# juhotuho10/rust_GPU_raytracing

Hardware: AMD Instinct MI355X
Metric: Mray/s (primary+bounce) at 1920x1080, 8 bounces; 1/2/4/8-GPU scaling (higher is better)
Workload: dtype f32

## Files before the change

include/rt_abi.h:

```cpp
#ifndef RT_ABI_H
#define RT_ABI_H

#include <stddef.h>
#include <stdint.h>

#ifdef __cplusplus
extern "C" {
#endif

#if defined(__GNUC__)
#define RT_API __attribute__((visibility("default")))
#else
#define RT_API
#endif

#define RT_ABI_VERSION 12

#define RT_OK 0
#define RT_E_INVALID -1
#define RT_E_HIP -2
#define RT_E_NOMEM -3
#define RT_E_CAPACITY -4
#define RT_E_NODEVICE -5

// ... 334 lines not shown
RT_API int rt_pack_owned_output(rt_ctx* ctx, void* dst_device);
RT_API int rt_unpack_output(rt_ctx* ctx, const void* src_device, uint32_t src_rank, uint32_t world_size);
RT_API int rt_unpack_accumulation_ranks(rt_ctx* ctx, const void* src_device, uint64_t stride_px,
                                        uint32_t world_size, uint32_t skip_rank, uint32_t divisor);
RT_API int rt_unpack_output_ranks(rt_ctx* ctx, const void* src_device, uint64_t stride_px, uint32_t world_size,
                                  uint32_t skip_rank);

RT_API int rt_launch_config(rt_ctx* ctx, uint32_t* threads, uint32_t* blocks, uint32_t* lds_bytes,
                            uint32_t* scene_in_lds);

#define RT_PASS_PATH 1u
#define RT_PASS_PRIMARY 2u
#define RT_PASS_RESOLVE 4u
#define RT_PASS_BRUTE 8u
#define RT_PASS_BRUTE_STREAM 16u
RT_API int rt_last_launch_passes(rt_ctx* ctx, uint32_t* passes);

RT_API int rt_debug_counters(rt_ctx* ctx, uint64_t* out, uint32_t n);

RT_API int rt_debug_check_leaf_certificates(rt_ctx* ctx, uint32_t* mismatches, uint32_t* valid, uint32_t* total);

RT_API int rt_math_selftest(uint32_t which, uint64_t* mismatches, uint32_t* first_bad);

RT_API void* rt_stream(rt_ctx* ctx);

RT_API int rt_srgb_table(float out[256]);

typedef struct rt_group rt_group;

RT_API int rt_create_multi(const rt_create_info* info, const int32_t* devices, uint32_t n_devices, rt_group** out);
// ... 72 lines not shown
```

rust_gpu_raytracing_amd/_native.py:

```python
from __future__ import annotations

import ctypes
import os
from pathlib import Path

import numpy as np

from . import buffers as B

LIB_NAME = "librt_pathtrace.so"
LIB_PATH = Path(__file__).resolve().parent / LIB_NAME

RT_OK = 0
RT_E_INVALID = -1
RT_E_HIP = -2
RT_E_NOMEM = -3
RT_E_CAPACITY = -4
RT_E_NODEVICE = -5

_ERR_NAMES = {
    RT_E_INVALID: "RT_E_INVALID",
    RT_E_HIP: "RT_E_HIP",
    RT_E_NOMEM: "RT_E_NOMEM",
    RT_E_CAPACITY: "RT_E_CAPACITY",
# ... 218 lines not shown
    "rt_group_update_triangles": (ctypes.c_int, [_P, _P, _U32]),
    "rt_group_update_object_info": (ctypes.c_int, [_P, _P, _U32]),
    "rt_group_update_sub_object_info": (ctypes.c_int, [_P, _P, _U32]),
    "rt_group_update_materials": (ctypes.c_int, [_P, _P, _U32]),
    "rt_group_upload_textures": (ctypes.c_int, [_P, _P, _U32, _U32, _U32]),
    "rt_group_upload_env_map": (ctypes.c_int, [_P, _P, _U32, _U32]),
    "rt_group_ray_count": (ctypes.c_int, [_P, ctypes.POINTER(ctypes.c_uint64)]),
    "rt_group_reset_ray_count": (ctypes.c_int, [_P]),
    "rt_gather_frame": (ctypes.c_int, [_P, _U32, _U32]),
    "rt_group_read_output": (ctypes.c_int, [_P, _U32, _P]),
    "rt_group_read_accumulation": (ctypes.c_int, [_P, _U32, _P]),
}

RT_DEFAULT_FRAME_BATCH = 16
RT_PASS_PATH, RT_PASS_PRIMARY, RT_PASS_RESOLVE, RT_PASS_BRUTE, RT_PASS_BRUTE_STREAM = 1, 2, 4, 8, 16
RT_GROUP_COPY_TRANSPORT = 1
RT_GATHER_IMAGE = 0
RT_GATHER_ACCUMULATION = 1
RT_DISPLAY_ACCUMULATION, RT_DISPLAY_DENOISED, RT_DISPLAY_PLANE = 0, 1, 2
RT_TONE_LINEAR, RT_TONE_REINHARD, RT_TONE_ACES = 0, 1, 2
RT_ENCODE_NONE, RT_ENCODE_SRGB = 0, 1

_lib = None


def load_library(path: os.PathLike | str | None = None) -> ctypes.CDLL:
    global _lib
    if path is None:
        if _lib is not None:
            return _lib
# ... 51 lines not shown
```

rust_gpu_raytracing_amd/csrc/pathtrace.hip:

```cpp
#include <hip/hip_runtime.h>
#include <stdint.h>

#include <algorithm>

#include "rt_path_common.h"
#include "rt_sphere_walk.h"
#include "rt_walk.h"

#ifdef RT_ISA_MARKS
#define RT_ISA_MARK(name) asm volatile("; RT_MARK " name)
#else
#define RT_ISA_MARK(name)
#endif

#pragma clang fp contract(off)

using namespace rtk;

constexpr uint32_t kPrimaryThreads = 1024;

constexpr uint32_t kQueueStride = 64;

__device__ __forceinline__ uint32_t* sched_orders(const KernelArgs& ka) { return ka.sched + 2u * ka.owned_tiles; }
__device__ __forceinline__ uint32_t* sched_flags(const KernelArgs& ka) { return ka.sched + 4u * ka.owned_tiles; }

__device__ __forceinline__ uint32_t xcc_id() {
    return __builtin_amdgcn_s_getreg((3 << 11) | (0 << 6) | 20);
}

struct TileQueue {
    uint32_t stripe;
    uint32_t empty;
// ... 16 lines not shown
            open = (uint64_t)v * n_str + st < ka.queue_units;
        }
        const uint64_t m = __ballot(open);
        if (m == 0) {
            q.empty = 1u;
            return 0xffffffffu;
        }
        uint32_t st = q.stripe + 1u + (uint32_t)__builtin_ctzll(m);
        q.stripe = st >= n_str ? st - n_str : st;
        if (lane == 0) old = atomicAdd(ka.queue + q.stripe * kQueueStride, 1u);
        pos = (uint64_t)__builtin_amdgcn_readlane(old, 0) * n_str + q.stripe;
        if (pos < ka.queue_units) return (uint32_t)pos;
    }
}

__device__ __forceinline__ uint32_t unit_tile(const KernelArgs& ka, uint32_t pos, uint32_t& frame) {
    if (pos == 0xffffffffu) return pos;
    uint32_t q;
    if (!ka.frame_light) {
        frame = 0u;
        q = pos;
    } else if (ka.unit_tile_major) {
        q = pos / ka.frames;
        frame = pos - q * ka.frames;
    } else {
        frame = pos / ka.owned_tiles;
        q = pos - frame * ka.owned_tiles;
    }
    return ka.tile_order ? ka.tile_order[q] : q;
}

__device__ __forceinline__ void record_tile_cost(uint32_t* cost, bool fin, uint32_t tile, uint32_t n) {
    uint64_t m = __ballot(fin);
    while (m) {
// ... 102 lines not shown
    unsigned long long* diag;
    __device__ __forceinline__ void operator()(bool walk, bool at_leaf, uint32_t) const {
        const uint64_t act = __ballot(walk), lf = __ballot(at_leaf);
        if (act && (threadIdx.x & 63u) == (uint32_t)__builtin_ctzll(__ballot(true))) {
            atomicAdd(diag + 22, 1ull);
            atomicAdd(diag + 23, (unsigned long long)__popcll(act));
            if (lf) {
                atomicAdd(diag + 24, 1ull);
                atomicAdd(diag + 25, (unsigned long long)__popcll(lf));
            }
        }
    }
};
#endif

template <int kMode, uint32_t kThreads, bool kTris>
__global__ void __launch_bounds__(kThreads, 1) rt_pathtrace_kernel(KernelArgs ka) {
    extern __shared__ __attribute__((aligned(16))) unsigned char lds[];
    __shared__ uint32_t block_rays;

    const uint32_t tid = threadIdx.x;
    if (ka.launch_clock && tid == 0) atomicMax(ka.launch_clock, ~(unsigned long long)wall_clock64());
    float* l_srgb = reinterpret_cast<float*>(lds + ka.lds_srgb_offset);
    SceneView sv{ka.sphere_slots, ka.sphere_orig, ka.sphere_material, ka.sphere_bvh, ka.materials, nullptr,
                 ka.objects,      l_srgb,         ka.tri_bvh,     ka.tri_prims, kTris ? *ka.tri_extent : 0.0f,
                 ka.sub_objects};
    if constexpr (kTris && kMode <= 1) {
        if (ka.tri_qnodes) {
            const float4 g0 = ka.tri_qgrid[0], g1 = ka.tri_qgrid[1];
            if (g0.w != 0.0f) {
                sv.tri_q = ka.tri_qnodes;
                sv.qox = g0.x;
                sv.qoy = g0.y;
                sv.qoz = g0.z;
                sv.qsx = g1.x;
                sv.qsy = g1.y;
// ... 48 lines not shown
        if (ka.lds_sub_offset) {
            RtSubObject* l_sub = reinterpret_cast<RtSubObject*>(lds + ka.lds_sub_offset);
            for (uint32_t i = tid; i < ka.sub_object_count; i += kThreads) l_sub[i] = ka.sub_objects[i];
            sv.sub = l_sub;
        }
    }
    for (uint32_t i = tid; i < 256u; i += kThreads) l_srgb[i] = ka.srgb[i];
    float* l_cam = l_srgb + 256;
    if (tid < 16u) {
        l_cam[tid] = ka.inv_proj[tid];
        l_cam[16u + tid] = ka.inv_view[tid];
    }
    if (tid == 0) l_cam[32] = ka.aspect;
    __syncthreads();

    const bool accumulate = ka.accumulate == 1u;
    const uint32_t samples = accumulate ? ka.compute_per_frame : 1u;

    constexpr uint32_t kIdle = 0, kSetup = 1, kTrav = 2, kDone = 3, kPrimary = 4;
    uint32_t rays = 0;
    uint32_t lane_tile = 0;
    uint32_t lane_slot = 0;
    const bool frame_par = ka.frame_light != nullptr;
    uint32_t mode = kIdle;
    uint32_t index = 0, sample = 0, frame = 0;
    float4 pix = make_float4(0.f, 0.f, 0.f, 0.f);
    Path p;
    p.o = p.d = mk(0.f, 0.f, 0.f);
    p.light = p.contrib = f4{0.f, 0.f, 0.f, 0.f};
    p.seed = p.bounce = 0;
    TraceState ts;
    ts.inv = mk(0.f, 0.f, 0.f);
    ts.a4 = ts.a2 = 0.f;
    ts.node = 0;
    ts.phase = 2;
    ts.nan_hit = false;
    ts.sph = SphereHit{kF32Max, 0u, 0u};
    ts.tri = TriHit{kF32Max, 0u, 0u, 0u, false};
// ... 8 lines not shown
        if (accumulate) {
            const float div = (float)((ka.accumulation_index + frame) * ka.compute_per_frame);
            r = clamp01(pix.x / div);
            g = clamp01(pix.y / div);
            b = clamp01(pix.z / div);
            a = clamp01(pix.w / div);
        } else {
            r = clamp01(p.light.x);
            g = clamp01(p.light.y);
            b = clamp01(p.light.z);
            a = clamp01(p.light.w);
        }
        if (accumulate) ka.accum[index] = pix;
        ka.output[index] = pack_rgba8(r, g, b, a);
    };
    auto finish_sample = [&]() {
        if (frame_par) {
            const size_t slot = (size_t)(frame * samples + sample) * ((size_t)ka.owned_tiles * 64u) +
                                (size_t)lane_tile * 64u + lane_slot;
            ka.frame_light[slot] = make_float4(p.light.x, p.light.y, p.light.z, p.light.w);
            sample += 1;
            if (sample < samples) {
                start_sample(ka, index, random_index(), pixel_ray(ka, l_cam, index, index % ka.width, index / ka.width),
                             p);
                mode = primary_start();
            } else {
                mode = kIdle;
            }
            return;
        }
        sample += 1;
        if (accumulate) {
            pix.x = pix.x + p.light.x;
            pix.y = pix.y + p.light.y;
            pix.z = pix.z + p.light.z;
            pix.w = pix.w + p.light.w;
        }
        if (sample == samples && frame + 1u < ka.frames) {
            store_frame();
            frame += 1;
            sample = 0;
        }
        if (sample < samples) {
            start_sample(ka, index, random_index(), pixel_ray(ka, l_cam, index, index % ka.width, index / ka.width), p);
            mode = primary_start();
        } else {
            store_frame();
            mode = kIdle;
        }
    };

#ifdef RT_DIAG_TAIL
    const unsigned long long wave_t0 = realtime();
    unsigned long long wave_dry = 0;
#endif
    if (blockIdx.x == 0 && threadIdx.x < ka.queue_stripes) ka.queue_next[threadIdx.x * kQueueStride] = 0u;
    TileQueue queue{(xcc_id() + 8u * (blockIdx.x >> 3)) % ka.queue_stripes, 0u};
    uint32_t tile_frame = 0;
    uint32_t tile = unit_tile(ka, claim_tile(ka, queue), tile_frame);
    uint32_t next = 0;
#ifdef RT_DIAG
    unsigned long long iters = 0, trav_cyc = 0, steps = 0, step_lanes = 0, shade_cyc = 0, refill_cyc = 0,
                       setup_cyc = 0, leaf_cyc = 0, leaf_steps = 0;
    unsigned long long shade_passes = 0, shade_lanes = 0, miss_lanes = 0, glass_lanes = 0, spec_lanes = 0,
                       setup_passes = 0, setup_lanes = 0;
    const unsigned long long t_start = stamp();
#endif
    while (true) {
#ifdef RT_DIAG
        ++iters;
        const unsigned long long ts0 = stamp();
#endif
        bool fin = false;
        uint32_t fin_rays = 0;
// ... 13 lines not shown
        }
#endif
        if (mode == kDone) {
            const Hit h = trace_end<kTris>(sv, ka, p.o, p.d, ts);
#ifdef RT_DIAG
            {
                const bool miss = h.t == kF32Max;
                const RtMaterial dmat = sv.mat[min(h.material_index, ka.material_count - 1u)];
                miss_lanes += (unsigned long long)__popcll(__ballot(miss));
                glass_lanes += (unsigned long long)__popcll(__ballot(!miss && dmat.glass > 0.0f));
                spec_lanes += (unsigned long long)__popcll(__ballot(!miss && !(dmat.glass > 0.0f) && dmat.specular > 0.0f));
            }
#endif
            ++rays;
            RT_ISA_MARK("shade");
            if (shade<(kMode >= 1)>(sv, ka, p, h)) {
                fin = true;
                fin_rays = p.bounce + (p.bounce < ka.bounces ? 1u : 0u);
                finish_sample();
            } else {
                mode = kSetup;
            }
        }
        if (ka.tile_cost) record_tile_cost(ka.tile_cost, fin, lane_tile, fin_rays);
#ifdef RT_DIAG
        const unsigned long long ts1 = stamp();
        shade_cyc += ts1 - ts0;
#endif
        RT_ISA_MARK("refill");
        while (true) {
            const uint64_t need = __ballot(mode == kIdle);
            if (need == 0 || tile >= ka.owned_tiles) break;
            const uint32_t avail = 64u - next;
            if (mode == kIdle) {
                const uint32_t rank =
                    __builtin_amdgcn_mbcnt_hi((uint32_t)(need >> 32), __builtin_amdgcn_mbcnt_lo((uint32_t)need, 0u));
                if (rank < avail) {
                    const uint32_t slot = next + rank;
                    const uint32_t gt = tile * ka.world_size + ka.rank;
                    const uint32_t x = (gt % ka.tiles_x) * 8u + (slot & 7u);
                    const uint32_t y = (gt / ka.tiles_x) * 8u + (slot >> 3);
                    if (x < ka.width && y < ka.height) {
                        index = y * ka.width + x;
                        lane_tile = tile;
                        lane_slot = slot;
                        sample = 0;
                        frame = tile_frame;
                        mode = kSetup;
                        if (accumulate && !frame_par) pix = ka.accum[index];
                        start_sample(ka, index, random_index(), pixel_ray(ka, l_cam, index, x, y), p);
                        mode = primary_start();
                    }
                }
            }
            next += min((uint32_t)__popcll(need), avail);
            if (next == 64u) {
                tile = unit_tile(ka, claim_tile(ka, queue), tile_frame);
                next = 0;
            #ifdef RT_DIAG_TAIL
                if (tile >= ka.owned_tiles && wave_dry == 0) wave_dry = realtime();
#endif
            }
        }
#ifdef RT_DIAG
        const unsigned long long ts2 = stamp();
        refill_cyc += ts2 - ts1;
#endif
#ifdef RT_DIAG
        {
            const uint64_t sm = __ballot(mode == kSetup);
            if (sm) {
                ++setup_passes;
                setup_lanes += (unsigned long long)__popcll(sm);
            }
        }
#endif
        RT_ISA_MARK("setup");
        if (mode == kSetup) {
            while (mode == kSetup && p.bounce >= ka.bounces) finish_sample();
            if (mode == kSetup) {
                trace_begin<kTris>(sv, ka, p.o, p.d, ts);
                mode = ts.phase == 2 ? kDone : kTrav;
            }
        }
#ifdef RT_DIAG
        setup_cyc += stamp() - ts2;
#endif
        if (__ballot(mode != kIdle) == 0 && tile >= ka.owned_tiles) break;
        const bool draining = tile >= ka.owned_tiles;
        uint32_t thresh = draining ? 0u : ka.trav_threshold;
        uint32_t n_active = 64u, min_steps = 0u;
        if constexpr (kDrainDecouple<kMode, kTris>) {
            if (draining) {
                thresh = ka.drain_threshold;
                n_active = (uint32_t)__popcll(__ballot(mode == kTrav || mode == kDone));
// ... 178 lines not shown
        if (tid == 0) {
            sorter = atomicAdd(sched_flags(ka) + par, 1u);
            if (blockIdx.x == 0) sched_flags(ka)[par ^ 1u] = 0u;
        }
        __syncthreads();
        if (sorter == 0)
            sort_tiles_by_cost<kThreads>(ka.sched + (par ^ 1u) * n, sched_orders(ka) + (par ^ 1u) * n, n,
                                         reinterpret_cast<uint32_t*>(lds + ka.lds_srgb_offset));
    }
    if (ka.launch_clock) {
        __syncthreads();
        if (tid == 0) atomicMax(ka.launch_clock + 1, (unsigned long long)wall_clock64());
    }
}

#define RT_FOR_EACH_CONFIG(X)                                                                                   \
    X(0, 256, true) X(0, 512, true) X(0, 1024, true) X(1, 256, true) X(1, 512, true) X(1, 1024, true)          \
    X(2, 256, true) X(2, 512, true) X(2, 1024, true) X(0, 256, false) X(0, 512, false) X(0, 1024, false)       \
    X(1, 256, false) X(1, 512, false) X(1, 1024, false)

constexpr uint32_t kBruteThreads = 256;

__device__ __forceinline__ void brute_sub_triangles(const KernelArgs& ka, f3 o, f3 d, uint32_t first_tri,
                                                    uint32_t count, uint32_t oi, float& closest, TriHit& best) {
    for (uint32_t j = 0; j < count; ++j) {
        const uint32_t ti = min(first_tri + j, ka.triangle_count - 1u);
        const TriGeom g = load_tri(ka.triangles, ti);
        const float det = -dot(d, g.cn);
        const float inv_det = 1.0f / det;
        const f3 ao = o - g.a;
        const float dist = dot(ao, g.cn) * inv_det;
        if (dist < 0.0f || dist >= closest) continue;
        const f3 dao = cross(ao, d);
        const float v = -dot(g.ab, dao) * inv_det;
// ... 510 lines not shown
            }();
    }
}

namespace {
hipError_t allow_big_lds(const void* fn) {
    int dev = 0, max_optin = 0;
    hipError_t e = hipGetDevice(&dev);
    if (e != hipSuccess) return e;
    e = hipDeviceGetAttribute(&max_optin, hipDeviceAttributeSharedMemPerBlockOptin, dev);
    if (e != hipSuccess || max_optin <= 0) return hipSuccess;
    return hipFuncSetAttribute(fn, hipFuncAttributeMaxDynamicSharedMemorySize, max_optin - 256);
}
}

hipError_t rt_launch_pathtrace(const KernelArgs& ka, int mode, bool tris, uint32_t threads, size_t lds_bytes,
                               uint32_t blocks, hipStream_t stream) {
#define RT_LAUNCH(M, T, TR)                                                                                    \
    if (mode == M && threads == T && tris == TR) {                                                            \
        hipLaunchKernelGGL((rt_pathtrace_kernel<M, T, TR>), dim3(blocks), dim3(T), lds_bytes, stream, ka);    \
        return hipGetLastError();                                                                             \
    }
    RT_FOR_EACH_CONFIG(RT_LAUNCH)
#undef RT_LAUNCH
    return hipErrorInvalidValue;
}

size_t rt_brute_wf_tile_bytes(bool stream) {
    if (stream) return (size_t)kBruteThreads * kBruteHits * 4u;
    return 2u * (size_t)kBruteWfTileSubs * sizeof(RtSubObject) + (size_t)kBruteThreads * kBruteRays * kBruteHits * 2u;
}

uint32_t rt_brute_wf_chunk() { return kBruteChunk; }

hipError_t rt_launch_brute_wf(const KernelArgs& ka, bool tris, bool scalar_stream, size_t lds_bytes, uint32_t blocks,
// ... 26 lines not shown
        if (lds_bytes > 64u * 1024u) {                                                                         \
            hipError_t e = allow_big_lds(reinterpret_cast<const void*>(&rt_primary_kernel<M, TR, T, W>));     \
            if (e != hipSuccess) return e;                                                                     \
        }                                                                                                      \
        hipLaunchKernelGGL((rt_primary_kernel<M, TR, T, W>), dim3(blocks), dim3(T), lds_bytes, stream, ka);   \
        return hipGetLastError();                                                                              \
    }
    RT_PRIMARY(1, true, 64, 0) RT_PRIMARY(1, true, 128, 0) RT_PRIMARY(1, true, 256, 0) RT_PRIMARY(1, true, 256, 8)
    RT_PRIMARY(1, true, 512, 0) RT_PRIMARY(1, true, 1024, 0) RT_PRIMARY(2, true, 1024, 0)
#undef RT_PRIMARY
    return hipErrorInvalidValue;
}

constexpr int kDefaultWavesPerCu = 16;

hipError_t rt_pathtrace_pick_config(int mode, bool tris, size_t lds_bytes, size_t lds_bytes_per_thread,
                                    uint32_t force_threads, uint32_t waves_cap, uint32_t* threads,
                                    int* blocks_per_cu) {
    const int kTargetWavesPerCu = waves_cap ? (int)waves_cap : kDefaultWavesPerCu;
    int best_waves = -1;
#define RT_OCC(M, T, TR)                                                                                  \
    if (mode == M && tris == TR) {                                                                        \
        int n = 0;                                                                                        \
        hipError_t e = allow_big_lds(reinterpret_cast<const void*>(&rt_pathtrace_kernel<M, T, TR>));     \
        if (e != hipSuccess) return e;                                                                    \
        e = hipOccupancyMaxActiveBlocksPerMultiprocessor(&n, rt_pathtrace_kernel<M, T, TR>, T,           \
                                                         lds_bytes + (size_t)T * lds_bytes_per_thread);  \
        if (e != hipSuccess) return e;                                                                    \
        const int waves = std::min(n * (int)(T / 64), kTargetWavesPerCu);                                 \
        if (n > 0 && (force_threads ? force_threads == T : waves > best_waves)) {                         \
            best_waves = waves;                                                                           \
            *threads = T;                                                                                 \
            *blocks_per_cu = force_threads ? n : std::max(1, std::min(n, kTargetWavesPerCu / (int)(T / 64))); \
        }                                                                                                 \
    }
    RT_FOR_EACH_CONFIG(RT_OCC)
#undef RT_OCC
    if (best_waves <= 0) return hipErrorInvalidConfiguration;
    return hipSuccess;
}

// ... 227 lines not shown
```

rust_gpu_raytracing_amd/csrc/rt_abi.cpp:

```cpp
#include <hip/hip_runtime.h>

#include <algorithm>
#include <cmath>
#include <cstddef>
#include <cstdio>
#include <cstdlib>
#include <cstring>
#include <initializer_list>
#include <new>
#include <string>
#include <vector>

#include "rt_abi.h"
#include "rt_kernel_args.h"
#include "rt_query_schedule.h"
#include "rt_scene_math.h"
#include "sphere_bvh.h"
#include "tri_cone.h"
#include "tri_qnode.h"

hipError_t rt_launch_math_selftest(uint32_t which, unsigned long long* mismatches, uint32_t* first_bad,
                                   hipStream_t stream);
hipError_t rt_launch_pathtrace(const KernelArgs& ka, int mode, bool tris, uint32_t threads, size_t lds_bytes,
                               uint32_t blocks, hipStream_t stream);
hipError_t rt_pathtrace_pick_config(int mode, bool tris, size_t lds_bytes, size_t lds_bytes_per_thread,
                                    uint32_t force_threads, uint32_t waves_cap, uint32_t* threads,
                                    int* blocks_per_cu);
hipError_t rt_launch_edit(const float* model, const uint32_t* tri_object, const uint32_t* sub_object,
                          const uint2* object_tris, const rt_scene::Placement* place, uint32_t object_count,
                          uint32_t n_tri, uint32_t n_sub, RtTriangleHot* tris, float4* bounds, RtSubObject* subs,
                          RtObject* objects, hipStream_t stream);
hipError_t rt_launch_quantize_tri_nodes(const SphereBvhNode* nodes, uint32_t n, const uint32_t* src,
                                        const uint32_t* skip, uint32_t n_out, SphereBvhNode* out32, uint4* q,
                                        float4* grid, hipStream_t stream);
hipError_t rt_launch_refit(SphereBvhNode* nodes, const SubObjectPrim* prims, const RtSubObject* subs,
                           const uint32_t* order, const uint32_t* level_offsets, uint32_t n_levels, float* extent_out,
                           hipStream_t stream);
hipError_t rt_launch_tri_leafcert(const SubObjectPrim* prims, uint32_t n_prims, const RtSubObject* subs,
                                  const RtTriangleHot* tris, uint32_t n_tri, TriLeafCert* out, hipStream_t stream);
hipError_t rt_launch_tri_leaftris(const SubObjectPrim* prims, uint32_t n_prims, const RtTriangleHot* tris,
                                  uint32_t n_tri, uint4* out, hipStream_t stream);
hipError_t rt_launch_primary(const KernelArgs& ka, int mode, bool tris, size_t lds_bytes, uint32_t threads,
// ... 144 lines not shown
    hipEvent_t ev_aux_done = nullptr;
    hipEvent_t ev_primary = nullptr;
    bool aux_outstanding = false;
    bool primary_dirty = true;
    uint64_t batches = 0;
    bool batch_overlap = true;
    bool stage_subs = true;
    size_t batch_budget = 0;
    bool use_qnodes = true;
    bool qnodes_dirty = true;
    bool derived_octants = false, derived_qnodes = false;
    uint4* d_tri_qnodes = nullptr;
    float4* d_tri_qgrid = nullptr;
    size_t qnodes_cap = 0;
    bool batch_schedule = false;
    bool unit_tile_major = true;

    uint32_t cap_mat = 0, cap_sph = 0, cap_tri = 0, cap_obj = 0, cap_sub = 0;
    uint32_t n_mat_dev = 1, n_tri_dev = 1, n_sub_dev = 1;

    float4* d_rays = nullptr;
    float4* d_accum = nullptr;
    uint32_t* d_out = nullptr;
    unsigned long long* d_counter = nullptr;
    uint32_t* d_queue = nullptr;
    uint32_t queue_parity[2] = {0, 0};
    uint32_t queue_stripes = kQueueStripes;
    int n_cu = 0;
    bool force_global_scene = false;
    size_t occ_lds_bytes = 0;
    int occ_mode = -1;
    bool occ_tris = false;
    size_t occ_stack_pt = 0;
    int max_lds_mode = 2;
    int occ_blocks_per_cu = 0;
    uint32_t occ_threads = 0;
    uint32_t force_threads = 0;
    uint32_t waves_cap = 0;
    uint32_t trav_threshold = 0;
    uint32_t drain_threshold = kDefaultDrainThreshold;
    uint32_t drain_min_steps = kDefaultDrainMinSteps;
    uint32_t leaf_batch = 0;
    uint32_t tile_schedule = kDefaultTileSchedule;
    uint32_t* d_tile_sched[2] = {};
    uint64_t sched_launches[2] = {};
    uint32_t last_blocks = 0, last_lds = 0;
    uint32_t last_passes = 0;
// ... 1053 lines not shown
        ka.tri_leaftris = ctx->d_tri_ltris;
    }
    if (sl.mode == 2) {
        ka.lds_srgb_offset = (uint32_t)(sl.mode2_bytes - kLdsTailBytes);
        sl.lds_bytes = sl.mode2_bytes;
    } else if (sl.mode == 1) {
        ka.lds_srgb_offset = (uint32_t)(sl.mode1_bytes - kLdsTailBytes);
        sl.lds_bytes = sl.mode1_bytes;
    } else {
        ka.lds_srgb_offset = 0;
        sl.lds_bytes = kLdsTailBytes;
    }
    return RT_OK;
}

static int dispatch_batch(rt_ctx* ctx, uint32_t bounces, uint32_t frames) {
    const rt_params& p = ctx->params;
    {
        int rc = refresh_sphere_slots(ctx, p.sphere_count, p.object_count == 0);
        if (rc) return rc;
        rc = refresh_tri_accel(ctx, p.object_count);
        if (rc) return rc;
    }
    KernelArgs ka{};
    ka.camera_rays = ctx->d_rays;
    ka.accum = ctx->d_accum;
    ka.output = ctx->d_out;
    ka.ray_counter = ctx->d_counter;
    ka.diag = ctx->d_counter + 1;
    ka.queue_stripes = ctx->queue_stripes;
// ... 22 lines not shown
            RT_HIP(ctx, join_aux(ctx));
            RT_HIP(ctx, hipStreamSynchronize(ctx->stream));
            for (float4*& b : ctx->d_frame_light) {
                if (b) RT_HIP(ctx, hipFree(b));
                b = nullptr;
            }
            ctx->frame_light_cap = 0;
            for (float4*& b : ctx->d_frame_light) {
                const hipError_t ea = hipMalloc(reinterpret_cast<void**>(&b), want * sizeof(float4));
                if (ea != hipSuccess) return fail(ctx, RT_E_NOMEM, std::string("frame lights: ") + hipGetErrorString(ea));
            }
            ctx->frame_light_cap = want;
        }
        ka.queue_units = ctx->owned_tiles * frames;
        ka.unit_tile_major = ctx->unit_tile_major ? 1u : 0u;
    }

    SceneLaunch sl;
    scene_carve(ctx, ka, ctx->force_global_scene ? 0 : ctx->max_lds_mode, sl);
    const bool tris = sl.tris;
    const int mode = sl.mode;
    if (ctx->brute) {
        scene_carve_layouts(ctx, ka, 1, kLdsSceneBudget, ctx->force_global_scene ? 0 : ctx->max_lds_mode, sl);
        ka.lds_srgb_offset = (uint32_t)(sl.mode1_bytes - kLdsTailBytes);
        ka.lds_stack_offset = (uint32_t)al16(sl.mode1_bytes);
        const uint32_t samples = ka.accumulate == 1u ? ka.compute_per_frame : 1u;
        const uint64_t passes = (uint64_t)frames * samples;
        const bool scalar_stream = tris && ctx->brute == 2;
        const size_t lds = ka.lds_stack_offset + rt_brute_wf_tile_bytes(scalar_stream);
        int dev = 0, max_optin = 0;
        RT_HIP(ctx, hipGetDevice(&dev));
// ... 47 lines not shown
        ctx->last_blocks = blocks;
        ctx->last_passes = RT_PASS_BRUTE | (scalar_stream ? RT_PASS_BRUTE_STREAM : 0u);
        ctx->last_lds = (uint32_t)lds;
        ctx->occ_threads = 256;
        ctx->primary_dirty = true;
        return RT_OK;
    }
    {
        const int rc = scene_accel_args(ctx, ka, sl);
        if (rc) return rc;
    }
    const bool coop = sl.coop;
    const size_t mode1_bytes = sl.mode1_bytes, mode2_bytes = sl.mode2_bytes;
    size_t lds_bytes = sl.lds_bytes;
    const size_t lane_pt = coop ? (size_t)kLeafBatchWaveBytes / 64u : 0u;
    if (ctx->occ_blocks_per_cu == 0 || ctx->occ_lds_bytes != lds_bytes || ctx->occ_mode != mode ||
        ctx->occ_tris != tris || ctx->occ_stack_pt != lane_pt) {
        int per_cu = 0;
        uint32_t threads = 0;
        hipError_t oe = rt_pathtrace_pick_config(mode, tris, lds_bytes, lane_pt, ctx->force_threads, ctx->waves_cap,
                                                 &threads, &per_cu);
        if (oe != hipSuccess) return hip_fail(ctx, "rt_pathtrace_pick_config (occupancy query)", oe);
        ctx->occ_blocks_per_cu = per_cu;
        ctx->occ_threads = threads;
        ctx->occ_lds_bytes = lds_bytes;
        ctx->occ_mode = mode;
        ctx->occ_tris = tris;
        ctx->occ_stack_pt = lane_pt;
    }
    ka.lds_leafbatch_offset = (uint32_t)al16(lds_bytes);
    if (coop) lds_bytes = ka.lds_leafbatch_offset + (size_t)ctx->occ_threads * lane_pt;
    const uint32_t waves_per_block = ctx->occ_threads / 64;
    const uint64_t resident = (uint64_t)ctx->occ_blocks_per_cu * (uint64_t)(ctx->n_cu > 0 ? ctx->n_cu : 1);
    const uint64_t wanted = ((uint64_t)ka.queue_units + waves_per_block - 1) / waves_per_block;
    const uint32_t blocks = (uint32_t)(wanted < resident ? wanted : resident);
    if (blocks == 0) return RT_OK;
    const bool sched = ctx->tile_schedule && (!frame_par || ctx->batch_schedule) &&
                       (uint64_t)ka.queue_units >= kSchedMinTilesPerWave * blocks * waves_per_block;
    const int si = (frame_par && ctx->batch_overlap) ? (int)(ctx->batches & 1u) : 0;
    hipStream_t S = si ? ctx->aux_stream : ctx->stream;
    if (!frame_par) RT_HIP(ctx, join_aux(ctx));
    if (si && ctx->primary_dirty) {
        RT_HIP(ctx, hipEventRecord(ctx->ev_primary, ctx->stream));
        RT_HIP(ctx, hipStreamWaitEvent(S, ctx->ev_primary, 0));
// ... 63 lines not shown
            for (uint4*& b : ctx->d_primary) {
                const hipError_t ea = hipMalloc(reinterpret_cast<void**>(&b), want * 16);
                if (ea != hipSuccess) return fail(ctx, RT_E_NOMEM, std::string("primary records: ") + hipGetErrorString(ea));
            }
            ctx->primary_cap = want;
        }
        KernelArgs pka = ka;
        pka.primary = ctx->d_primary[pi];
        pka.queue_units = ctx->owned_tiles * frames;
        pka.primary_tile_major = ctx->primary_tile_major ? 1u : 0u;
        const size_t image = mode == 2 ? mode2_bytes : mode1_bytes;
        const uint32_t min_waves = (mode == 2 || ctx->primary_threads != 256u) ? 0u : ctx->primary_min_waves;
        RT_HIP(ctx, rt_launch_primary(pka, mode, tris, image, mode == 2 ? 1024u : ctx->primary_threads, min_waves, S));
        ka.primary = pka.primary;
    }
    hipError_t e = rt_launch_pathtrace(ka, mode, tris, ctx->occ_threads, lds_bytes, blocks, S);
    ctx->last_blocks = blocks;
    ctx->last_passes = RT_PASS_PATH | (primary ? RT_PASS_PRIMARY : 0u) | (frame_par ? RT_PASS_RESOLVE : 0u);
    ctx->last_lds = (uint32_t)lds_bytes;
    if (e != hipSuccess) return hip_fail(ctx, "rt_pathtrace_kernel launch", e);
    if (frame_par) {
        if (ctx->batches > 0) RT_HIP(ctx, hipStreamWaitEvent(S, ctx->ev_resolved[(ctx->batches - 1) & 1u], 0));
        e = rt_launch_resolve(ctx->d_accum, ctx->d_out, ka.frame_light, ctx->width, ctx->height, ctx->tiles_x,
                              ctx->owned_tiles, ctx->rank, ctx->world, p.accumulation_index, p.compute_per_frame,
                              frames, ka.launch_clock ? ka.launch_clock + 2 : nullptr, S);
        if (e != hipSuccess) return hip_fail(ctx, "rt_resolve_frames_kernel launch", e);
        RT_HIP(ctx, hipEventRecord(ctx->ev_resolved[ctx->batches & 1u], S));
        ctx->batches += 1;
    }
    ctx->queue_parity[si] ^= 1u;
    if (si) {
        RT_HIP(ctx, hipEventRecord(ctx->ev_aux_done, S));
        ctx->aux_outstanding = true;
// ... 998 lines not shown
        if ((rc = range(0, 63)) == RT_OK) ctx->drain_threshold = (uint32_t)v;
    } else if (k == "drain_min_steps") {
        if ((rc = range(0, 1 << 20)) == RT_OK) ctx->drain_min_steps = (uint32_t)v;
    } else if (k == "leaf_batch") {
        if ((rc = range(0, 8)) == RT_OK) ctx->leaf_batch = (uint32_t)v;
    } else if (k == "tile_schedule") {
        if ((rc = range(0, 1)) == RT_OK) ctx->tile_schedule = (uint32_t)v;
    } else if (k == "frame_parallel") {
        rc = flag(ctx->frame_parallel);
    } else if (k == "batch_overlap") {
        rc = flag(ctx->batch_overlap);
    } else if (k == "batch_schedule") {
        rc = flag(ctx->batch_schedule);
    } else if (k == "unit_tile_major") {
        rc = flag(ctx->unit_tile_major);
    } else if (k == "query_chunk") {
        if ((rc = range(1, (int32_t)kMaxQueryChunk)) == RT_OK) ctx->query_chunk = (uint32_t)v;
    } else if (k == "gather_chunk") {
        if ((rc = range(1, (int32_t)kMaxGatherChunk)) == RT_OK) ctx->gather_chunk = (uint32_t)v;
    } else if (k == "query_lds_mode") {
        if ((rc = range(-1, 2)) == RT_OK) ctx->query_lds_mode = v;
    } else if (k == "feature_band") {
        if ((rc = range(64, (int32_t)kMaxFeatureBand)) == RT_OK) ctx->feature_band = (uint32_t)v;
    } else if (k == "denoise_lds") {
        rc = flag(ctx->denoise_lds);
    } else if (k == "batch_memory_mb") {
        if ((rc = range(1, 1 << 30)) == RT_OK) ctx->batch_budget = (size_t)v << 20;
    } else {
        return fail(ctx, RT_E_INVALID, "rt_set_tuning: unknown key " + k);
    }
// ... 271 lines not shown
```

rust_gpu_raytracing_amd/csrc/rt_kernel_args.h:

```cpp
#pragma once
#include <hip/hip_runtime.h>
#include <stdint.h>

#include "tri_cone.h"

struct RtSphere {
    float position[3];
    float radius;
    uint32_t material_index;
    uint32_t _pad[3];
};

struct RtMaterial {
    uint32_t texture_index;
    float roughness;
    float emission_power;
    float specular;
    float specular_scatter;
    float glass;
    float refraction_index;
    uint32_t _pad;
};

struct RtObject {
// ... 147 lines not shown
    uint32_t drain_min_steps;
    uint32_t leaf_batch;
    uint32_t queue_stripes;
    uint32_t sched_bits;
    uint32_t lds_mat_offset;
    uint32_t lds_mat_aux_offset;
    uint32_t lds_obj_offset;
    uint32_t lds_orig_offset;
    uint32_t lds_smat_offset;
    uint32_t lds_nodes_offset;
    uint32_t lds_tri_nodes_offset;
    uint32_t lds_tri_prims_offset;
    uint32_t lds_sub_offset;
    uint32_t lds_stack_offset;
    uint32_t lds_srgb_offset;
};
```

rust_gpu_raytracing_amd/csrc/rt_path_common.h:

```cpp
#pragma once
#include <hip/hip_runtime.h>
#include <stdint.h>

#include "rt_bvh_slab.h"
#include "rt_device_math.h"
#include "rt_kernel_args.h"
#include "rt_sphere_roots.h"
#include "tri_qnode.h"

#pragma clang fp contract(off)

using namespace rtk;

namespace {

struct Hit {
    float t;
    f3 p;
    f3 n;
    uint32_t material_index;
    bool front_face;
    float u, v;
};

// ... 268 lines not shown
    }
    return h;
}

struct HitId {
    uint32_t kind, index, triangle;
};
template <bool kTris>
__device__ __forceinline__ HitId trace_end_id(const TraceState& ts) {
    const float tt = (kTris && ts.tri.t != kF32Max) ? ts.tri.t : kF32Max;
    if (ts.sph.t < tt) return HitId{1u, ts.sph.orig, 0u};
    if (kTris && ts.tri.t != kF32Max) return HitId{2u, ts.tri.obj, ts.tri.tri};
    return HitId{0u, 0u, 0u};
}

__device__ __forceinline__ uint32_t fetch_texture(const KernelArgs& ka, uint32_t layer, float u, float v) {
    const int x = texel_coord(u * (float)(int32_t)ka.texture_width, ka.tex_w);
    const int y = texel_coord(v * (float)(int32_t)ka.texture_height, ka.tex_h);
    const uint32_t l = min(layer, ka.tex_layers - 1u);
    const size_t off = ((size_t)l * ka.tex_h + (size_t)y) * ka.tex_w + (size_t)x;
    return ka.textures[off];
}

__device__ __forceinline__ f4 sample_env(const KernelArgs& ka, const float* srgb, f3 d) {
    int x = 0, y = 0;
    if (!(ka.env_uniform & 1u)) {
        const float u = 0.5f + div_const(atan2f_c(d.z, d.x), kTwoPiWgsl, kInvTwoPiWgsl);
        x = texel_coord(u * (float)(int32_t)ka.env_map_width, ka.env_w);
    }
    if (!(ka.env_uniform & 2u)) {
        const float v = 0.5f + div_const(asinf_c(d.y), kWgslPi, kInvWgslPi);
        y = texel_coord(v * (float)(int32_t)ka.env_map_height, ka.env_h);
    }
    return decode_texel(ka.env[(size_t)y * ka.env_w + (size_t)x], srgb);
}

struct Path {
    f3 o, d;
    f4 light, contrib;
// ... 42 lines not shown
    p.bounce = 0;
}

__device__ __forceinline__ void start_sample_at(f3 origin, uint32_t stream, uint32_t random_index, f3 dir, Path& p) {
    p.o = origin;
    p.d = dir;
    p.seed = stream * random_index * 326624u;
    const float rx = random01(p.seed), ry = random01(p.seed), rz = random01(p.seed);
    const f3 jit = mk(rx * 2.0f - 1.0f, ry * 2.0f - 1.0f, rz * 2.0f - 1.0f);
    p.d = p.d + jit * 0.0005f;
    p.contrib = f4{1.0f, 1.0f, 1.0f, 1.0f};
    p.light = f4{0.0f, 0.0f, 0.0f, 0.0f};
    p.bounce = 0;
}

template <bool kAux>
__device__ __forceinline__ bool shade(const SceneView& sv, const KernelArgs& ka, Path& p, const Hit& h) {
    if (h.t == kF32Max) {
        const f4 c = sample_env(ka, sv.srgb, p.d);
        p.light.x = p.light.x + c.x * p.contrib.x;
        p.light.y = p.light.y + c.y * p.contrib.y;
        p.light.z = p.light.z + c.z * p.contrib.z;
        p.light.w = p.light.w + c.w * p.contrib.w;
        return true;
    }
    const uint32_t mi = min(h.material_index, ka.material_count - 1u);
    const RtMaterial m = sv.mat[mi];
    const bool tex1 = kAux && ka.tex_w == 1u && ka.tex_h == 1u;
    uint32_t texel = 0;
    if (!tex1) texel = fetch_texture(ka, m.texture_index, h.u, h.v);
    const float gx = normal01(p.seed);
    const float gy = normal01(p.seed);
// ... 147 lines not shown
```

rust_gpu_raytracing_amd/renderer.py:

```python
from __future__ import annotations

import ctypes

import numpy as np

from . import _native as N
from . import buffers as B
from .scene import RenderScene

REFERENCE_BOUNCES = 10


class Renderer:
    def __init__(
        self,
        scene: RenderScene,
        *,
        accumulate: bool = True,
        compute_per_frame: int = 1,
        device: int = 0,
        rank: int = 0,
        world_size: int = 1,
        camera_rays: np.ndarray | None = None,
        device_rays: bool | None = None,
# ... 604 lines not shown
        self._call("rt_set_tile_schedule", schedule)

    def tile_schedule_state(self):
        n = self.owned_pixel_count() // 64
        order = np.zeros(n, np.uint32)
        costs = np.zeros(n, np.uint32)
        self._call("rt_tile_schedule_state", order.ctypes.data_as(ctypes.c_void_p),
                   costs.ctypes.data_as(ctypes.c_void_p))
        return order, costs

    def launch_config(self) -> dict:
        v = [ctypes.c_uint32() for _ in range(4)]
        N.check(self._ctx, self._lib.rt_launch_config(self._ctx, *[ctypes.byref(x) for x in v]), self._lib)
        return dict(zip(("threads", "blocks", "lds_bytes", "scene_in_lds"), (x.value for x in v)))

    def last_launch_passes(self) -> list:
        v = ctypes.c_uint32()
        N.check(self._ctx, self._lib.rt_last_launch_passes(self._ctx, ctypes.byref(v)), self._lib)
        names = ((N.RT_PASS_PATH, "path"), (N.RT_PASS_PRIMARY, "primary"), (N.RT_PASS_RESOLVE, "resolve"),
                 (N.RT_PASS_BRUTE, "brute"), (N.RT_PASS_BRUTE_STREAM, "brute_stream"))
        return [n for bit, n in names if v.value & bit]

    @property
    def stream_handle(self) -> int:
        return self._lib.rt_stream(self._ctx) or 0

    def close(self) -> None:
        if self._ctx is not None:
            self._lib.rt_destroy(self._ctx)
            self._ctx = None

    def __enter__(self):
        return self
# ... 10 lines not shown
```

Before: 25470.

## Add frame-parallel path-trace kernel instance with kernarg-reloaded shade args

Adds a compile-time frame-parallel variant of the path-tracing kernel, selected by default when frame-parallel batching, accumulation and at least one bounce are active. It drops the runtime accumulate, frame_par and bounce-limit checks from the hot loop. Shading arguments are re-read from the kernarg segment at each shade through an opaque pointer, so they need not stay live in scalar registers across traversal. The light-plane stride becomes a kernel argument, and occupancy results are cached separately per variant. This doubles the number of kernel instantiations, and the early bounce-limit loop in setup is removed for this variant.

```diff
diff --git a/include/rt_abi.h b/include/rt_abi.h
--- a/include/rt_abi.h
+++ b/include/rt_abi.h
@@ -372,6 +372,7 @@
 #define RT_PASS_RESOLVE 4u
 #define RT_PASS_BRUTE 8u
 #define RT_PASS_BRUTE_STREAM 16u
+#define RT_PASS_PATH_FRAME_PAR 64u
 RT_API int rt_last_launch_passes(rt_ctx* ctx, uint32_t* passes);
 
 RT_API int rt_debug_counters(rt_ctx* ctx, uint64_t* out, uint32_t n);
diff --git a/rust_gpu_raytracing_amd/_native.py b/rust_gpu_raytracing_amd/_native.py
--- a/rust_gpu_raytracing_amd/_native.py
+++ b/rust_gpu_raytracing_amd/_native.py
@@ -256,6 +256,7 @@
 
 RT_DEFAULT_FRAME_BATCH = 16
 RT_PASS_PATH, RT_PASS_PRIMARY, RT_PASS_RESOLVE, RT_PASS_BRUTE, RT_PASS_BRUTE_STREAM = 1, 2, 4, 8, 16
+RT_PASS_PATH_FRAME_PAR = 64
 RT_GROUP_COPY_TRANSPORT = 1
 RT_GATHER_IMAGE = 0
 RT_GATHER_ACCUMULATION = 1
diff --git a/rust_gpu_raytracing_amd/csrc/pathtrace.hip b/rust_gpu_raytracing_amd/csrc/pathtrace.hip
--- a/rust_gpu_raytracing_amd/csrc/pathtrace.hip
+++ b/rust_gpu_raytracing_amd/csrc/pathtrace.hip
@@ -16,6 +16,22 @@
 #pragma clang fp contract(off)
 
 using namespace rtk;
+
+typedef const __attribute__((address_space(4))) unsigned char* KernargPtr;
+__device__ __forceinline__ KernargPtr kernarg_fresh(KernargPtr kp) {
+    asm volatile("" : "+s"(kp));
+    return kp;
+}
+#define RT_KERNARG(kp, field)                                                                        \
+    (*reinterpret_cast<const __attribute__((address_space(4))) decltype(KernelArgs::field)*>(        \
+        (kp) + __builtin_offsetof(KernelArgs, field)))
+__device__ __forceinline__ ShadeArgs load_shade_args(KernargPtr kp) {
+    return ShadeArgs{RT_KERNARG(kp, textures),        RT_KERNARG(kp, env),           RT_KERNARG(kp, texture_width),
+                     RT_KERNARG(kp, texture_height),  RT_KERNARG(kp, env_map_width), RT_KERNARG(kp, env_map_height),
+                     RT_KERNARG(kp, material_count),  RT_KERNARG(kp, tex_w),         RT_KERNARG(kp, tex_h),
+                     RT_KERNARG(kp, tex_layers),      RT_KERNARG(kp, env_w),         RT_KERNARG(kp, env_h),
+                     RT_KERNARG(kp, env_uniform),     RT_KERNARG(kp, bounces)};
+}
 
 constexpr uint32_t kPrimaryThreads = 1024;
 
@@ -62,10 +78,11 @@
     }
 }
 
+template <bool kFramePar>
 __device__ __forceinline__ uint32_t unit_tile(const KernelArgs& ka, uint32_t pos, uint32_t& frame) {
     if (pos == 0xffffffffu) return pos;
     uint32_t q;
-    if (!ka.frame_light) {
+    if (!kFramePar && !ka.frame_light) {
         frame = 0u;
         q = pos;
     } else if (ka.unit_tile_major) {
@@ -198,12 +215,13 @@
 };
 #endif
 
-template <int kMode, uint32_t kThreads, bool kTris>
+template <int kMode, uint32_t kThreads, bool kTris, bool kFramePar>
 __global__ void __launch_bounds__(kThreads, 1) rt_pathtrace_kernel(KernelArgs ka) {
     extern __shared__ __attribute__((aligned(16))) unsigned char lds[];
     __shared__ uint32_t block_rays;
 
     const uint32_t tid = threadIdx.x;
+    const KernargPtr kernarg = (KernargPtr)__builtin_amdgcn_kernarg_segment_ptr();
     if (ka.launch_clock && tid == 0) atomicMax(ka.launch_clock, ~(unsigned long long)wall_clock64());
     float* l_srgb = reinterpret_cast<float*>(lds + ka.lds_srgb_offset);
     SceneView sv{ka.sphere_slots, ka.sphere_orig, ka.sphere_material, ka.sphere_bvh, ka.materials, nullptr,
@@ -282,14 +300,14 @@
     if (tid == 0) l_cam[32] = ka.aspect;
     __syncthreads();
 
-    const bool accumulate = ka.accumulate == 1u;
+    const bool accumulate = kFramePar || ka.accumulate == 1u;
     const uint32_t samples = accumulate ? ka.compute_per_frame : 1u;
 
     constexpr uint32_t kIdle = 0, kSetup = 1, kTrav = 2, kDone = 3, kPrimary = 4;
     uint32_t rays = 0;
     uint32_t lane_tile = 0;
     uint32_t lane_slot = 0;
-    const bool frame_par = ka.frame_light != nullptr;
+    const bool frame_par = kFramePar || ka.frame_light != nullptr;
     uint32_t mode = kIdle;
     uint32_t index = 0, sample = 0, frame = 0;
     float4 pix = make_float4(0.f, 0.f, 0.f, 0.f);
@@ -328,39 +346,46 @@
         if (accumulate) ka.accum[index] = pix;
         ka.output[index] = pack_rgba8(r, g, b, a);
     };
+    auto finish_sample_frame_par = [&]() {
+        const size_t plane = kFramePar ? (size_t)ka.light_plane : (size_t)ka.owned_tiles * 64u;
+        const size_t slot = (size_t)(frame * samples + sample) * plane + (size_t)lane_tile * 64u + lane_slot;
+        ka.frame_light[slot] = make_float4(p.light.x, p.light.y, p.light.z, p.light.w);
+        sample += 1;
+        if (sample < samples) {
+            start_sample(ka, index, random_index(), pixel_ray(ka, l_cam, index, index % ka.width, index / ka.width), p);
+            mode = primary_start();
+        } else {
+            mode = kIdle;
+        }
+    };
     auto finish_sample = [&]() {
-        if (frame_par) {
-            const size_t slot = (size_t)(frame * samples + sample) * ((size_t)ka.owned_tiles * 64u) +
-                                (size_t)lane_tile * 64u + lane_slot;
-            ka.frame_light[slot] = make_float4(p.light.x, p.light.y, p.light.z, p.light.w);
+        if constexpr (kFramePar) {
+            finish_sample_frame_par();
+        } else {
+            if (frame_par) {
+                finish_sample_frame_par();
+                return;
+            }
             sample += 1;
+            if (accumulate) {
+                pix.x = pix.x + p.light.x;
+                pix.y = pix.y + p.light.y;
+                pix.z = pix.z + p.light.z;
+                pix.w = pix.w + p.light.w;
+            }
+            if (sample == samples && frame + 1u < ka.frames) {
+                store_frame();
+                frame += 1;
+                sample = 0;
+            }
             if (sample < samples) {
                 start_sample(ka, index, random_index(), pixel_ray(ka, l_cam, index, index % ka.width, index / ka.width),
                              p);
                 mode = primary_start();
             } else {
+                store_frame();
                 mode = kIdle;
             }
-            return;
-        }
-        sample += 1;
-        if (accumulate) {
-            pix.x = pix.x + p.light.x;
-            pix.y = pix.y + p.light.y;
-            pix.z = pix.z + p.light.z;
-            pix.w = pix.w + p.light.w;
-        }
-        if (sample == samples && frame + 1u < ka.frames) {
-            store_frame();
-            frame += 1;
-            sample = 0;
-        }
-        if (sample < samples) {
-            start_sample(ka, index, random_index(), pixel_ray(ka, l_cam, index, index % ka.width, index / ka.width), p);
-            mode = primary_start();
-        } else {
-            store_frame();
-            mode = kIdle;
         }
     };
 
@@ -371,7 +396,7 @@
     if (blockIdx.x == 0 && threadIdx.x < ka.queue_stripes) ka.queue_next[threadIdx.x * kQueueStride] = 0u;
     TileQueue queue{(xcc_id() + 8u * (blockIdx.x >> 3)) % ka.queue_stripes, 0u};
     uint32_t tile_frame = 0;
-    uint32_t tile = unit_tile(ka, claim_tile(ka, queue), tile_frame);
+    uint32_t tile = unit_tile<kFramePar>(ka, claim_tile(ka, queue), tile_frame);
     uint32_t next = 0;
 #ifdef RT_DIAG
     unsigned long long iters = 0, trav_cyc = 0, steps = 0, step_lanes = 0, shade_cyc = 0, refill_cyc = 0,
@@ -415,9 +440,19 @@
 #endif
             ++rays;
             RT_ISA_MARK("shade");
-            if (shade<(kMode >= 1)>(sv, ka, p, h)) {
+            bool ended;
+            uint32_t bounce_limit;
+            if constexpr (kFramePar) {
+                const ShadeArgs sa = load_shade_args(kernarg_fresh(kernarg));
+                ended = shade<(kMode >= 1)>(sv, sa, p, h);
+                bounce_limit = sa.bounces;
+            } else {
+                ended = shade<(kMode >= 1)>(sv, ka, p, h);
+                bounce_limit = ka.bounces;
+            }
+            if (ended) {
                 fin = true;
-                fin_rays = p.bounce + (p.bounce < ka.bounces ? 1u : 0u);
+                fin_rays = p.bounce + (p.bounce < bounce_limit ? 1u : 0u);
                 finish_sample();
             } else {
                 mode = kSetup;
@@ -448,7 +483,7 @@
                         sample = 0;
                         frame = tile_frame;
                         mode = kSetup;
-                        if (accumulate && !frame_par) pix = ka.accum[index];
+                        if (!kFramePar && accumulate && !frame_par) pix = ka.accum[index];
                         start_sample(ka, index, random_index(), pixel_ray(ka, l_cam, index, x, y), p);
                         mode = primary_start();
                     }
@@ -456,7 +491,7 @@
             }
             next += min((uint32_t)__popcll(need), avail);
             if (next == 64u) {
-                tile = unit_tile(ka, claim_tile(ka, queue), tile_frame);
+                tile = unit_tile<kFramePar>(ka, claim_tile(ka, queue), tile_frame);
                 next = 0;
             #ifdef RT_DIAG_TAIL
                 if (tile >= ka.owned_tiles && wave_dry == 0) wave_dry = realtime();
@@ -478,8 +513,9 @@
 #endif
         RT_ISA_MARK("setup");
         if (mode == kSetup) {
-            while (mode == kSetup && p.bounce >= ka.bounces) finish_sample();
-            if (mode == kSetup) {
+            if constexpr (!kFramePar)
+                while (mode == kSetup && p.bounce >= ka.bounces) finish_sample();
+            if (kFramePar || mode == kSetup) {
                 trace_begin<kTris>(sv, ka, p.o, p.d, ts);
                 mode = ts.phase == 2 ? kDone : kTrav;
             }
@@ -688,10 +724,11 @@
     }
 }
 
-#define RT_FOR_EACH_CONFIG(X)                                                                                   \
-    X(0, 256, true) X(0, 512, true) X(0, 1024, true) X(1, 256, true) X(1, 512, true) X(1, 1024, true)          \
-    X(2, 256, true) X(2, 512, true) X(2, 1024, true) X(0, 256, false) X(0, 512, false) X(0, 1024, false)       \
-    X(1, 256, false) X(1, 512, false) X(1, 1024, false)
+#define RT_FOR_EACH_SHAPE(X, FP)                                                                                \
+    X(0, 256, true, FP) X(0, 512, true, FP) X(0, 1024, true, FP) X(1, 256, true, FP) X(1, 512, true, FP)       \
+    X(1, 1024, true, FP) X(2, 256, true, FP) X(2, 512, true, FP) X(2, 1024, true, FP) X(0, 256, false, FP)     \
+    X(0, 512, false, FP) X(0, 1024, false, FP) X(1, 256, false, FP) X(1, 512, false, FP) X(1, 1024, false, FP)
+#define RT_FOR_EACH_CONFIG(X) RT_FOR_EACH_SHAPE(X, false) RT_FOR_EACH_SHAPE(X, true)
 
 constexpr uint32_t kBruteThreads = 256;
 
@@ -1232,11 +1269,12 @@
 }
 }
 
-hipError_t rt_launch_pathtrace(const KernelArgs& ka, int mode, bool tris, uint32_t threads, size_t lds_bytes,
-                               uint32_t blocks, hipStream_t stream) {
-#define RT_LAUNCH(M, T, TR)                                                                                    \
-    if (mode == M && threads == T && tris == TR) {                                                            \
-        hipLaunchKernelGGL((rt_pathtrace_kernel<M, T, TR>), dim3(blocks), dim3(T), lds_bytes, stream, ka);    \
+hipError_t rt_launch_pathtrace(const KernelArgs& ka, int mode, bool tris, bool frame_par, uint32_t threads,
+                               size_t lds_bytes, uint32_t blocks, hipStream_t stream) {
+    if (frame_par && (!ka.frame_light || ka.accumulate != 1u || ka.bounces == 0)) return hipErrorInvalidValue;
+#define RT_LAUNCH(M, T, TR, FP)                                                                                \
+    if (mode == M && threads == T && tris == TR && frame_par == FP) {                                         \
+        hipLaunchKernelGGL((rt_pathtrace_kernel<M, T, TR, FP>), dim3(blocks), dim3(T), lds_bytes, stream, ka); \
         return hipGetLastError();                                                                             \
     }
     RT_FOR_EACH_CONFIG(RT_LAUNCH)
@@ -1293,17 +1331,17 @@
 
 constexpr int kDefaultWavesPerCu = 16;
 
-hipError_t rt_pathtrace_pick_config(int mode, bool tris, size_t lds_bytes, size_t lds_bytes_per_thread,
-                                    uint32_t force_threads, uint32_t waves_cap, uint32_t* threads,
-                                    int* blocks_per_cu) {
+hipError_t rt_pathtrace_pick_config(int mode, bool tris, bool frame_par, size_t lds_bytes,
+                                    size_t lds_bytes_per_thread, uint32_t force_threads, uint32_t waves_cap,
+                                    uint32_t* threads, int* blocks_per_cu) {
     const int kTargetWavesPerCu = waves_cap ? (int)waves_cap : kDefaultWavesPerCu;
     int best_waves = -1;
-#define RT_OCC(M, T, TR)                                                                                  \
-    if (mode == M && tris == TR) {                                                                        \
+#define RT_OCC(M, T, TR, FP)                                                                              \
+    if (mode == M && tris == TR && frame_par == FP) {                                                     \
         int n = 0;                                                                                        \
-        hipError_t e = allow_big_lds(reinterpret_cast<const void*>(&rt_pathtrace_kernel<M, T, TR>));     \
+        hipError_t e = allow_big_lds(reinterpret_cast<const void*>(&rt_pathtrace_kernel<M, T, TR, FP>)); \
         if (e != hipSuccess) return e;                                                                    \
-        e = hipOccupancyMaxActiveBlocksPerMultiprocessor(&n, rt_pathtrace_kernel<M, T, TR>, T,           \
+        e = hipOccupancyMaxActiveBlocksPerMultiprocessor(&n, rt_pathtrace_kernel<M, T, TR, FP>, T,       \
                                                          lds_bytes + (size_t)T * lds_bytes_per_thread);  \
         if (e != hipSuccess) return e;                                                                    \
         const int waves = std::min(n * (int)(T / 64), kTargetWavesPerCu);                                 \
diff --git a/rust_gpu_raytracing_amd/csrc/rt_abi.cpp b/rust_gpu_raytracing_amd/csrc/rt_abi.cpp
--- a/rust_gpu_raytracing_amd/csrc/rt_abi.cpp
+++ b/rust_gpu_raytracing_amd/csrc/rt_abi.cpp
@@ -21,11 +21,11 @@
 
 hipError_t rt_launch_math_selftest(uint32_t which, unsigned long long* mismatches, uint32_t* first_bad,
                                    hipStream_t stream);
-hipError_t rt_launch_pathtrace(const KernelArgs& ka, int mode, bool tris, uint32_t threads, size_t lds_bytes,
-                               uint32_t blocks, hipStream_t stream);
-hipError_t rt_pathtrace_pick_config(int mode, bool tris, size_t lds_bytes, size_t lds_bytes_per_thread,
-                                    uint32_t force_threads, uint32_t waves_cap, uint32_t* threads,
-                                    int* blocks_per_cu);
+hipError_t rt_launch_pathtrace(const KernelArgs& ka, int mode, bool tris, bool frame_par, uint32_t threads,
+                               size_t lds_bytes, uint32_t blocks, hipStream_t stream);
+hipError_t rt_pathtrace_pick_config(int mode, bool tris, bool frame_par, size_t lds_bytes,
+                                    size_t lds_bytes_per_thread, uint32_t force_threads, uint32_t waves_cap,
+                                    uint32_t* threads, int* blocks_per_cu);
 hipError_t rt_launch_edit(const float* model, const uint32_t* tri_object, const uint32_t* sub_object,
                           const uint2* object_tris, const rt_scene::Placement* place, uint32_t object_count,
                           uint32_t n_tri, uint32_t n_sub, RtTriangleHot* tris, float4* bounds, RtSubObject* subs,
@@ -200,6 +200,7 @@
     float4* d_tri_qgrid = nullptr;
     size_t qnodes_cap = 0;
     bool batch_schedule = false;
+    bool frame_par_instance = true;
     bool unit_tile_major = true;
 
     uint32_t cap_mat = 0, cap_sph = 0, cap_tri = 0, cap_obj = 0, cap_sub = 0;
@@ -217,6 +218,12 @@
     size_t occ_lds_bytes = 0;
     int occ_mode = -1;
     bool occ_tris = false;
+    struct OccEntry {
+        size_t lds_bytes = 0, stack_pt = 0;
+        int mode = -1, blocks_per_cu = 0;
+        bool tris = false;
+        uint32_t threads = 0, force_threads = 0, waves_cap = 0;
+    } occ_cache[2];
     size_t occ_stack_pt = 0;
     int max_lds_mode = 2;
     int occ_blocks_per_cu = 0;
@@ -1300,6 +1307,10 @@
     return RT_OK;
 }
 
+static bool rt_path_frame_par_instance(bool frame_par_batch, uint32_t accumulate, uint32_t bounces, bool enabled) {
+    return enabled && frame_par_batch && accumulate == 1u && bounces >= 1u;
+}
+
 static int dispatch_batch(rt_ctx* ctx, uint32_t bounces, uint32_t frames) {
     const rt_params& p = ctx->params;
     {
@@ -1352,7 +1363,9 @@
         }
         ka.queue_units = ctx->owned_tiles * frames;
         ka.unit_tile_major = ctx->unit_tile_major ? 1u : 0u;
-    }
+        ka.light_plane = (uint32_t)owned_px;
+    }
+    const bool fp_instance = rt_path_frame_par_instance(frame_par, p.accumulate, bounces, ctx->frame_par_instance);
 
     SceneLaunch sl;
     scene_carve(ctx, ka, ctx->force_global_scene ? 0 : ctx->max_lds_mode, sl);
@@ -1430,20 +1443,29 @@
     const size_t mode1_bytes = sl.mode1_bytes, mode2_bytes = sl.mode2_bytes;
     size_t lds_bytes = sl.lds_bytes;
     const size_t lane_pt = coop ? (size_t)kLeafBatchWaveBytes / 64u : 0u;
-    if (ctx->occ_blocks_per_cu == 0 || ctx->occ_lds_bytes != lds_bytes || ctx->occ_mode != mode ||
-        ctx->occ_tris != tris || ctx->occ_stack_pt != lane_pt) {
+    rt_ctx::OccEntry& oc = ctx->occ_cache[fp_instance ? 1 : 0];
+    if (oc.blocks_per_cu == 0 || oc.lds_bytes != lds_bytes || oc.mode != mode || oc.tris != tris ||
+        oc.stack_pt != lane_pt || oc.force_threads != ctx->force_threads || oc.waves_cap != ctx->waves_cap) {
         int per_cu = 0;
         uint32_t threads = 0;
-        hipError_t oe = rt_pathtrace_pick_config(mode, tris, lds_bytes, lane_pt, ctx->force_threads, ctx->waves_cap,
-                                                 &threads, &per_cu);
+        hipError_t oe = rt_pathtrace_pick_config(mode, tris, fp_instance, lds_bytes, lane_pt, ctx->force_threads,
+                                                 ctx->waves_cap, &threads, &per_cu);
         if (oe != hipSuccess) return hip_fail(ctx, "rt_pathtrace_pick_config (occupancy query)", oe);
-        ctx->occ_blocks_per_cu = per_cu;
-        ctx->occ_threads = threads;
-        ctx->occ_lds_bytes = lds_bytes;
-        ctx->occ_mode = mode;
-        ctx->occ_tris = tris;
-        ctx->occ_stack_pt = lane_pt;
-    }
+        oc.blocks_per_cu = per_cu;
+        oc.threads = threads;
+        oc.lds_bytes = lds_bytes;
+        oc.mode = mode;
+        oc.tris = tris;
+        oc.stack_pt = lane_pt;
+        oc.force_threads = ctx->force_threads;
+        oc.waves_cap = ctx->waves_cap;
+    }
+    ctx->occ_blocks_per_cu = oc.blocks_per_cu;
+    ctx->occ_threads = oc.threads;
+    ctx->occ_lds_bytes = lds_bytes;
+    ctx->occ_mode = mode;
+    ctx->occ_tris = tris;
+    ctx->occ_stack_pt = lane_pt;
     ka.lds_leafbatch_offset = (uint32_t)al16(lds_bytes);
     if (coop) lds_bytes = ka.lds_leafbatch_offset + (size_t)ctx->occ_threads * lane_pt;
     const uint32_t waves_per_block = ctx->occ_threads / 64;
@@ -1537,9 +1559,10 @@
         RT_HIP(ctx, rt_launch_primary(pka, mode, tris, image, mode == 2 ? 1024u : ctx->primary_threads, min_waves, S));
         ka.primary = pka.primary;
     }
-    hipError_t e = rt_launch_pathtrace(ka, mode, tris, ctx->occ_threads, lds_bytes, blocks, S);
+    hipError_t e = rt_launch_pathtrace(ka, mode, tris, fp_instance, ctx->occ_threads, lds_bytes, blocks, S);
     ctx->last_blocks = blocks;
-    ctx->last_passes = RT_PASS_PATH | (primary ? RT_PASS_PRIMARY : 0u) | (frame_par ? RT_PASS_RESOLVE : 0u);
+    ctx->last_passes = RT_PASS_PATH | (primary ? RT_PASS_PRIMARY : 0u) | (frame_par ? RT_PASS_RESOLVE : 0u) |
+                       (fp_instance ? RT_PASS_PATH_FRAME_PAR : 0u);
     ctx->last_lds = (uint32_t)lds_bytes;
     if (e != hipSuccess) return hip_fail(ctx, "rt_pathtrace_kernel launch", e);
     if (frame_par) {
@@ -2568,6 +2591,8 @@
         rc = flag(ctx->batch_schedule);
     } else if (k == "unit_tile_major") {
         rc = flag(ctx->unit_tile_major);
+    } else if (k == "frame_par_instance") {
+        rc = flag(ctx->frame_par_instance);
     } else if (k == "query_chunk") {
         if ((rc = range(1, (int32_t)kMaxQueryChunk)) == RT_OK) ctx->query_chunk = (uint32_t)v;
     } else if (k == "gather_chunk") {
diff --git a/rust_gpu_raytracing_amd/csrc/rt_kernel_args.h b/rust_gpu_raytracing_amd/csrc/rt_kernel_args.h
--- a/rust_gpu_raytracing_amd/csrc/rt_kernel_args.h
+++ b/rust_gpu_raytracing_amd/csrc/rt_kernel_args.h
@@ -185,4 +185,5 @@
     uint32_t lds_sub_offset;
     uint32_t lds_stack_offset;
     uint32_t lds_srgb_offset;
+    uint32_t light_plane;
 };
diff --git a/rust_gpu_raytracing_amd/csrc/rt_path_common.h b/rust_gpu_raytracing_amd/csrc/rt_path_common.h
--- a/rust_gpu_raytracing_amd/csrc/rt_path_common.h
+++ b/rust_gpu_raytracing_amd/csrc/rt_path_common.h
@@ -306,7 +306,16 @@
     return HitId{0u, 0u, 0u};
 }
 
-__device__ __forceinline__ uint32_t fetch_texture(const KernelArgs& ka, uint32_t layer, float u, float v) {
+struct ShadeArgs {
+    const uint32_t* __restrict__ textures;
+    const uint32_t* __restrict__ env;
+    uint32_t texture_width, texture_height, env_map_width, env_map_height, material_count;
+    uint32_t tex_w, tex_h, tex_layers, env_w, env_h, env_uniform;
+    uint32_t bounces;
+};
+
+template <class KA>
+__device__ __forceinline__ uint32_t fetch_texture(const KA& ka, uint32_t layer, float u, float v) {
     const int x = texel_coord(u * (float)(int32_t)ka.texture_width, ka.tex_w);
     const int y = texel_coord(v * (float)(int32_t)ka.texture_height, ka.tex_h);
     const uint32_t l = min(layer, ka.tex_layers - 1u);
@@ -314,7 +323,8 @@
     return ka.textures[off];
 }
 
-__device__ __forceinline__ f4 sample_env(const KernelArgs& ka, const float* srgb, f3 d) {
+template <class KA>
+__device__ __forceinline__ f4 sample_env(const KA& ka, const float* srgb, f3 d) {
     int x = 0, y = 0;
     if (!(ka.env_uniform & 1u)) {
         const float u = 0.5f + div_const(atan2f_c(d.z, d.x), kTwoPiWgsl, kInvTwoPiWgsl);
@@ -387,8 +397,8 @@
     p.bounce = 0;
 }
 
-template <bool kAux>
-__device__ __forceinline__ bool shade(const SceneView& sv, const KernelArgs& ka, Path& p, const Hit& h) {
+template <bool kAux, class KA>
+__device__ __forceinline__ bool shade(const SceneView& sv, const KA& ka, Path& p, const Hit& h) {
     if (h.t == kF32Max) {
         const f4 c = sample_env(ka, sv.srgb, p.d);
         p.light.x = p.light.x + c.x * p.contrib.x;
diff --git a/rust_gpu_raytracing_amd/renderer.py b/rust_gpu_raytracing_amd/renderer.py
--- a/rust_gpu_raytracing_amd/renderer.py
+++ b/rust_gpu_raytracing_amd/renderer.py
@@ -642,9 +642,13 @@
         N.check(self._ctx, self._lib.rt_launch_config(self._ctx, *[ctypes.byref(x) for x in v]), self._lib)
         return dict(zip(("threads", "blocks", "lds_bytes", "scene_in_lds"), (x.value for x in v)))
 
-    def last_launch_passes(self) -> list:
+    def last_launch_pass_mask(self) -> int:
         v = ctypes.c_uint32()
         N.check(self._ctx, self._lib.rt_last_launch_passes(self._ctx, ctypes.byref(v)), self._lib)
+        return v.value
+
+    def last_launch_passes(self) -> list:
+        v = ctypes.c_uint32(self.last_launch_pass_mask())
         names = ((N.RT_PASS_PATH, "path"), (N.RT_PASS_PRIMARY, "primary"), (N.RT_PASS_RESOLVE, "resolve"),
                  (N.RT_PASS_BRUTE, "brute"), (N.RT_PASS_BRUTE_STREAM, "brute_stream"))
         return [n for bit, n in names if v.value & bit]
```

Result: faster. 26220 (median of 6 runs) (+2.9%).
